# atlas-jj/ORB-SLAM-free-space-carving

Hardware: AMD Instinct MI355X
Metric: Mpix*KF/s fused (640x480xN_KF) (higher is better)
Workload: dtype f32

## Files before the change

orb-slam-free-space-carving_amd/csrc/sdm_device.h:

```cpp
#pragma once
#include <hip/hip_runtime.h>
#include <float.h>
#include <stddef.h>
#include <stdint.h>

#include "sdm_c.h"

namespace sdm {

struct KfMeta {
    float fx, fy, cx, cy;
    float Tcw[12];
    float I_stddev;
    int uploaded;
    int pad[2];
};

struct RefConst {
    int slot;
    float fx, fy, cx, cy;
    float mind, maxd;
    int act_count;
};

// ... 182 lines not shown
    const float u1 = fx * x_min / z_min + cx;
    const float u2 = fx * x_max / z_max + cx;
    const float cols = (float)W;
    const float umin = __builtin_amdgcn_fmed3f(fminf(u1, u2), 0.0f, cols);
    const float umax = __builtin_amdgcn_fmed3f(fmaxf(u1, u2), 0.0f, cols);
    lo = (int)ceilf(umin);
    hi = (int)floorf(umax);
    return !__builtin_isunordered(u1, u2);
}

__device__ __forceinline__ bool gate2_fails_ref(float d, float lambdaL)
{
    if (d >= 360) d -= 360;
    if (d < 0) d += 360;
    if (d > 180) d = 360 - d;
    if (d > 90) d = 180 - d;
    return d > lambdaL;
}
__device__ __forceinline__ bool gate3_fails_ref(float d, float lambdaTheta)
{
    if (d >= 360) d -= 360;
    if (d < 0) d += 360;
    if (d > 180) d = 360 - d;
    return d > lambdaTheta;
}
__device__ __forceinline__ float wrap_neg360(float d)
{
    unsigned neg = (unsigned)((int)__float_as_uint(d) >> 31);
    return d + __uint_as_float(neg & 0x43B40000u);
}
__device__ __forceinline__ bool gate2_fails_fast(float d)
{
    float x = wrap_neg360(d);
    return (fabsf(x - 90.0f) < 10.0f) | (fabsf(x - 270.0f) < 10.0f);
}
__device__ __forceinline__ bool gate3_fails_fast(float d)
{
    float x = wrap_neg360(d);
    return (x > 45.0f) & (x < 315.0f);
}
__device__ __forceinline__ bool gate2_fails_k(float d, float g2c)
{
    const float x = wrap_neg360(d);
    return fabsf(fabsf(x - 180.0f) - 90.0f) < g2c;
}
__device__ __forceinline__ bool gate3_fails_k(float d, unsigned g3lo, unsigned g3span)
{
    const float x = wrap_neg360(d);
    return (__float_as_uint(x) - g3lo) < g3span;
}
__device__ __forceinline__ bool gate2_fails_fast1(float d)
{
    const float x = wrap_neg360(d);
    return fabsf(fabsf(x - 180.0f) - 90.0f) < 10.0f;
}
__device__ __forceinline__ bool gate3_fails_fast1(float d)
{
    const float x = wrap_neg360(d);
    return (__float_as_uint(x) - 0x42340001u) < (0x439D8000u - 0x42340001u);
}

__device__ __forceinline__ float match_cost(float pe2, float ge2, const DevParams& prm)
{
    double s = (double)pe2 + (double)ge2 * prm.inv_theta;
    unsigned lo = (unsigned)__double2loint(s);
    bool risky = (((lo & 0x1FFFFFFFu) - 0x0FFFFF00u) <= 0x200u) | !(s > 1.0e-30) | !(s < 1.0e30);
    if (__builtin_expect(risky, 0)) s = (double)pe2 + (double)ge2 / prm.theta_var;
    return (float)s;
}

#ifndef SDM_ABLATE
#define SDM_ABLATE 0
#endif
#ifndef SDM_SCAN_UNROLL
#define SDM_SCAN_UNROLL 4
#endif
constexpr int SCAN_UNROLL = SDM_SCAN_UNROLL;
typedef float v4f __attribute__((ext_vector_type(4)));

struct SearchStats {
    unsigned long long searches, candidates, gate_pass;
};

__device__ __forceinline__ float rcp_exact(float b)
{
    const float ab = fabsf(b);
    if (__builtin_expect(!((ab >= 0x1p-125f) & (ab < 0x1p125f)), 0)) return 1.0f / b;
    const float r = __builtin_amdgcn_rcpf(b);
    const float e = __builtin_fmaf(-b, r, 1.0f);
    return __builtin_fmaf(e, r, r);
}

#ifndef SDM_K1_OPT_ATAN_RCP
#define SDM_K1_OPT_ATAN_RCP 1
#endif
__device__ __forceinline__ float fast_atan2_deg_x1(float y)
{
    const float scale = (float)(180.0 / 3.14159265358979323846);
    const float p1 = 0.9997878412794807f * scale;
    const float p3 = -0.3258083974640975f * scale;
    const float p5 = 0.1555786518463281f * scale;
    const float p7 = -0.04432655554792128f * scale;
    float ay = fabsf(y);
    float a, c, c2;
    if (1.0f >= ay) {
        c = ay;
        c2 = c * c;
        a = (((p7 * c2 + p5) * c2 + p3) * c2 + p1) * c;
    } else {
#if SDM_K1_OPT_ATAN_RCP
        c = rcp_exact(ay + (float)DBL_EPSILON);
#else
        c = 1.0f / (ay + (float)DBL_EPSILON);
#endif
        c2 = c * c;
        a = 90.f - (((p7 * c2 + p5) * c2 + p3) * c2 + p1) * c;
    }
    if (y < 0) a = 360.f - a;
    return a;
}

#ifndef SDM_K1_OPT
#define SDM_K1_OPT 0x3a27f
#endif

constexpr int PCV_FLOATS = 20;
constexpr int CV_RX = 9, CV_RZ = 12, CV_TX = 15, CV_TZ = 16, CV_ROT = 17, CV_ISTD = 18;
static_assert(offsetof(PairConst, Rx) == 4 * CV_RX && offsetof(PairConst, Rz) == 4 * CV_RZ && offsetof(PairConst, tx) == 4 * CV_TX &&
                  offsetof(PairConst, tz) == 4 * CV_TZ && offsetof(PairConst, rot) == 4 * CV_ROT &&
                  offsetof(PairConst, istd) == 4 * CV_ISTD && offsetof(PairConst, Ry) == 4 * PCV_FLOATS,
              "the CV_* indices follow PairConst");

__device__ __forceinline__ float match_cost1(float pe2, float ge2, const DevParams& prm)
{
    double s = (double)pe2 + (double)ge2 * prm.inv_theta;
    const unsigned lo = (unsigned)__double2loint(s), hi = (unsigned)__double2hiint(s);
    const bool risky = (((lo & 0x1FFFFFFFu) - 0x0FFFFF00u) <= 0x200u) | ((hi - 0x39C00000u) >= (0x46200000u - 0x39C00000u));
    if (__builtin_expect(risky, 0)) s = (double)pe2 + (double)ge2 / prm.theta_var;
    return (float)s;
}

constexpr float INV_THETA_DEFAULT_F = (float)(1.0 / 0.23);
constexpr unsigned COST_BAND = 16u;
__device__ __forceinline__ float match_cost_ref(float pe2, float ge2, const DevParams& prm)
{
    return (float)((double)pe2 + (double)ge2 / prm.theta_var);
}
__device__ __forceinline__ float match_cost_approx(float pe2, float ge2) { return __builtin_fmaf(ge2, INV_THETA_DEFAULT_F, pe2); }

__device__ __forceinline__ float lerp_w0(float yf)
{
#if SDM_K1_OPT & 0x10
    return 1.0f - __builtin_amdgcn_fractf(yf);
#else
    return (floorf(yf) + 1.0f) - yf;
#endif
}
__device__ __forceinline__ float rec_lerp_im_w(const float4& r, float y0w)
{
    unsigned w = __float_as_uint(r.w);
    float y1w = 1.0f - y0w;
    float v0 = (float)(int)(w & 0xffu), v1 = (float)(int)((w >> 8) & 0xffu);
    return v0 * y0w + v1 * y1w;
}
__device__ __forceinline__ float rec_lerp_grad_w(const float4& r, float y0w)
{
    float y1w = 1.0f - y0w;
    return r.x * y0w + r.z * y1w;
}

__device__ __forceinline__ int cvt_i32_sat(float x)
{
    int r;
    asm("v_cvt_i32_f32 %0, %1" : "=v"(r) : "v"(x));
    return r;
}
__device__ __forceinline__ bool search_range_int1(float fx, float cx, float rxxp, float rzxp, float tx, float tz,
                                                  float mind, float maxd, int W, int& lo, int& hi)
{
    float x_min = rxxp * mind + tx, z_min = rzxp * mind + tz;
    float x_max = rxxp * maxd + tx, z_max = rzxp * maxd + tz;
    const float u1 = fx * x_min / z_min + cx;
    const float u2 = fx * x_max / z_max + cx;
    const float mn = __builtin_amdgcn_fmed3f(u1, u2, -__builtin_inff());
    const float mx = __builtin_amdgcn_fmed3f(u1, u2, __builtin_inff());
    lo = min(max(cvt_i32_sat(ceilf(mn)), 0), W);
    hi = min(max(cvt_i32_sat(floorf(mx)), 0), W - 1);
// ... 67 lines not shown
    }
    return ok;
}

struct ScanState {
    float old_err, best_pe, best_ge;
    int best_pixel;
};

struct ScanConst {
    const char* nbase;
    unsigned W16;
    float hlim_b;
    float ab, cb, pixel, grad1, th_line, ang_pi_rot, gate_lim;
    int hi;
};
template <bool STATS, bool CLEAN>
__device__ __forceinline__ void scan_candidate(const ScanConst& q, int uj, float yf, const float4& r, const DevParams& prm,
                                               ScanState& S, SearchStats* st)
{
    if (r.x < prm.lambdaG) return;
#if SDM_ABLATE == 4
    if (r.z > S.old_err) { S.best_pixel = uj; S.old_err = r.z; }
    return;
#endif
    const float d2 = r.y - q.th_line;
    const float d3 = r.y - q.ang_pi_rot;
    bool fail;
    if (CLEAN) {
#if SDM_K1_OPT & 0x04
        fail = gate2_fails_fast1(d2) | gate3_fails_fast1(d3);
#else
        fail = gate2_fails_fast(d2) | gate3_fails_fast(d3);
#endif
    } else {
        fail = gate2_fails_k(d2, prm.g2c) | gate3_fails_k(d3, prm.g3lo, prm.g3span);
        if (__builtin_expect(!((d2 < q.gate_lim) & (d3 < q.gate_lim)), 0))
            fail = gate2_fails_ref(d2, prm.lambdaL) || gate3_fails_ref(d3, prm.lambdaTheta);
    }
    if (fail) return;
    if (STATS) st->gate_pass++;
#if SDM_ABLATE == 3 || SDM_ABLATE == 4
    if (r.z > S.old_err) { S.best_pixel = uj; S.old_err = r.z; }
    return;
#endif
    const float y0w = lerp_w0(yf);
    float pe = q.pixel - rec_lerp_im_w(r, y0w);
    float ge = q.grad1 - rec_lerp_grad_w(r, y0w);
#if SDM_K1_OPT & 0x2000
    if (CLEAN || prm.approx_ok) {
        const float e = CLEAN ? match_cost_approx(pe * pe, ge * ge) : __builtin_fmaf(ge * ge, prm.inv_theta_f, pe * pe);
        bool better = e < S.old_err;
        if (__builtin_expect((__float_as_uint(e) - __float_as_uint(S.old_err) + COST_BAND) <= 2u * COST_BAND, 0))
            better = match_cost_ref(pe * pe, ge * ge, prm) < match_cost_ref(S.best_pe * S.best_pe, S.best_ge * S.best_ge, prm);
        if (better) {
#if SDM_K1_OPT & 0x4000
            asm volatile("" ::: "memory");
#endif
            S.best_pixel = uj;
            S.old_err = e;
            S.best_pe = pe;
            S.best_ge = ge;
        }
        return;
    }
#endif
#if SDM_K1_OPT & 0x08
    float err = match_cost1(pe * pe, ge * ge, prm);
#else
    float err = match_cost(pe * pe, ge * ge, prm);
#endif
    if (err < S.old_err) {
        S.best_pixel = uj;
        S.old_err = err;
        S.best_pe = pe;
        S.best_ge = ge;
    }
}

template <bool STATS, bool CLEAN, int NB>
__device__ __forceinline__ void scan_batch(const ScanConst& q, int u0, float u0f, const DevParams& prm, ScanState& S,
                                           SearchStats* st)
{
    float yfs[NB];
    unsigned long long rowok[NB];
    v4f rs[NB];
    const unsigned c0 = (unsigned)u0 << 4;
#if !(SDM_K1_OPT & 0x01)
    const unsigned hi16 = (unsigned)max(q.hi, 0) << 4;
#endif
#pragma unroll
    for (int k = 0; k < NB; k++) {
        float yf = -(q.ab * (u0f + (float)k) + q.cb);
        float yc = __builtin_amdgcn_fmed3f(yf, 1.0f, q.hlim_b);
#if SDM_K1_OPT & 0x01
        const unsigned off = __umul24((unsigned)(int)yc, q.W16) + c0;
        const char* __restrict__ nb_k = q.nbase + 16 * k;
#else
        unsigned uc16 = min(c0 + 16u * k, hi16);
        unsigned off = __umul24((unsigned)(int)yc, q.W16) + uc16;
        const char* __restrict__ nb_k = q.nbase;
#endif
        yfs[k] = yf;
        rowok[k] = __builtin_amdgcn_fcmpf(yc, yf, 1 );
#if SDM_ABLATE == 5
        rs[k] = v4f{20.0f + (float)(off & 15u), 10.0f, 21.0f, __uint_as_float(0x6040u)};
#else
        rs[k] = *reinterpret_cast<const v4f*>(nb_k + off);
#endif
    }
#pragma unroll
    for (int k = 0; k < NB; k++)
        asm volatile("" : "+v"(rs[k]));
#pragma unroll
    for (int k = 0; k < NB; k++) {
        const int uj = u0 + k;
        if (STATS && uj <= q.hi) st->candidates++;
        const float4 r = make_float4(rs[k].x, rs[k].y, rs[k].z, rs[k].w);
        if (!((uj <= q.hi) & __builtin_amdgcn_inverse_ballot_w64(rowok[k]))) continue;
        scan_candidate<STATS, CLEAN>(q, uj, yfs[k], r, prm, S, st);
    }
}

template <bool STATS, bool CLEAN>
__device__ __forceinline__ void scan_segment(const ScanConst& q, int lo, const DevParams& prm, ScanState& S, SearchStats* st)
{
    float u0f = (float)lo;
    for (int u0 = lo; u0 <= q.hi; u0 += SCAN_UNROLL, u0f += (float)SCAN_UNROLL)
        scan_batch<STATS, CLEAN, SCAN_UNROLL>(q, u0, u0f, prm, S, st);
}

#ifndef SDM_MASK_MIN_L
#define SDM_MASK_MIN_L 24
#endif
#ifndef SDM_MASK_MIN_L_UNION
#define SDM_MASK_MIN_L_UNION 48
#endif
#ifndef SDM_MASK_MAX_SLOPE
#define SDM_MASK_MAX_SLOPE 0.25f
#endif
#ifndef SDM_MASK_NB
#define SDM_MASK_NB 2
#endif
#ifndef SDM_MASK_BINS
#define SDM_MASK_BINS 1
#endif
constexpr int MASK_BINS = 16;
constexpr int MASK_WINDOW = 6;
constexpr int MASK_UNION = MASK_BINS + MASK_WINDOW - 1;
constexpr int MASK_PLANES = MASK_UNION + 1;
constexpr unsigned MASK_WORD_BYTES = 4u * MASK_PLANES;
constexpr float MASK_EPS = 0x1p-6f;
constexpr int MASK_HINT_L = SDM_MASK_MIN_L * 3 / 4;
#ifndef SDM_MASK_CALL_MEAN_L
#define SDM_MASK_CALL_MEAN_L 32
#endif
constexpr int MASK_CALL_MEAN_L = SDM_MASK_CALL_MEAN_L;
constexpr float MASK_ANG_MARGIN = 0.01f;
constexpr float MASK_MAX_LAMBDA_THETA = 56.0f;
constexpr float MASK_BIN_SCALE = (float)MASK_BINS / 360.0f;
__host__ __device__ __forceinline__ int mask_bin(float t)
{
    const int b = (int)(t * MASK_BIN_SCALE);
    return b < MASK_BINS - 1 ? b : MASK_BINS - 1;
}
struct MaskStats {
    unsigned long long waves, steps, row_mismatch;
};
struct MaskView {
    const char* base;
    unsigned row_pitch;
};
template <bool STATS, bool CLEAN, bool BINNED>
__device__ __forceinline__ void scan_masked(const ScanConst& q, const MaskView& mv, int lo, const DevParams& prm, ScanState& S,
                                            SearchStats* st, MaskStats* ms)
{
    const float yh = -(q.ab * (float)q.hi + q.cb);
    const float inv_s = __builtin_amdgcn_rcpf(fabsf(q.ab)) * 0.998046875f;
    const bool falling = q.ab > 0.0f;
    unsigned pl0 = 4u * (unsigned)MASK_UNION;
    if (BINNED) {
        float w0 = q.ang_pi_rot - (prm.lambdaTheta + MASK_ANG_MARGIN);
        if (w0 < 0.0f) w0 += 360.0f;
        pl0 = 4u * (unsigned)mask_bin(w0);
    }
    for (int base = lo; base <= q.hi; base += 64) {
        const int chi = min(q.hi, base + 63);
        unsigned long long cand = 0ull;
        bool ended = false;
        int u = base;
        while (u <= chi) {
            const float yf = -(q.ab * (float)u + q.cb);
            const float yc = __builtin_amdgcn_fmed3f(yf, 1.0f, q.hlim_b);
            if (!(yc == yf)) {
                const bool out_lo = (yf < 1.0f) & (yh < 1.0f), out_hi = (yf > q.hlim_b) & (yh > q.hlim_b);
                if (!(yf == yf) | out_lo | out_hi) {
                    if (STATS) st->candidates += (unsigned long long)(q.hi - u + 1);
                    ended = true;
                    break;
                }
                if (STATS) st->candidates++;
                u++;
                continue;
            }
            const float fr = __builtin_amdgcn_fractf(yf);
            const float room = (falling ? fr : 1.0f - fr) - MASK_EPS;
            const int n = max(cvt_i32_sat(room * inv_s), 0);
            const int cover = min(min(n, chi - u), 32);
            const char* __restrict__ mp = mv.base + (__umul24((unsigned)(int)yc, mv.row_pitch) + __umul24((unsigned)u >> 5, MASK_WORD_BYTES) + pl0);
            unsigned mlo, mhi;
            if (BINNED) {
                typedef unsigned mword4 __attribute__((ext_vector_type(4), aligned(4)));
                typedef unsigned mword2 __attribute__((ext_vector_type(2), aligned(4)));
                const mword4 a0 = *reinterpret_cast<const mword4*>(mp);
                const mword2 a1 = *reinterpret_cast<const mword2*>(mp + 16);
                const mword4 b0 = *reinterpret_cast<const mword4*>(mp + MASK_WORD_BYTES);
                const mword2 b1 = *reinterpret_cast<const mword2*>(mp + MASK_WORD_BYTES + 16);
                mlo = (a0.x | a0.y | a0.z) | (a0.w | a1.x | a1.y);
                mhi = (b0.x | b0.y | b0.z) | (b0.w | b1.x | b1.y);
            } else {
                mlo = *reinterpret_cast<const unsigned*>(mp);
                mhi = *reinterpret_cast<const unsigned*>(mp + MASK_WORD_BYTES);
            }
            unsigned long long bits = (((unsigned long long)mhi << 32) | (unsigned long long)mlo) >> ((unsigned)u & 31u);
            bits &= (2ull << cover) - 1ull;
            cand |= bits << (unsigned)(u - base);
            if (STATS) {
                st->candidates += (unsigned long long)(cover + 1);
                ms->steps++;
            }
            u += cover + 1;
        }
        if (STATS) {
            for (int k = 0; base + k <= (ended ? u - 1 : chi); k++) {
                const float yk = -(q.ab * (float)(base + k) + q.cb);
                if (!(__builtin_amdgcn_fmed3f(yk, 1.0f, q.hlim_b) == yk)) continue;
                const v4f r = *reinterpret_cast<const v4f*>(q.nbase + (__umul24((unsigned)(int)yk, q.W16) + ((unsigned)(base + k) << 4)));
                if (r.x < prm.lambdaG) continue;
                const bool fail = gate2_fails_ref(r.y - q.th_line, prm.lambdaL) || gate3_fails_ref(r.y - q.ang_pi_rot, prm.lambdaTheta);
                if (!fail && !((cand >> k) & 1ull)) ms->row_mismatch++;
            }
        }
        while (cand != 0ull) {
            int ujs[SDM_MASK_NB];
            float yfs[SDM_MASK_NB];
            v4f rs[SDM_MASK_NB];
            unsigned long long okm[SDM_MASK_NB];
#pragma unroll
            for (int k = 0; k < SDM_MASK_NB; k++) {
                okm[k] = __builtin_amdgcn_ballot_w64(cand != 0ull);
                const int uj = base + (cand != 0ull ? (int)__builtin_ctzll(cand) : 0);
                cand &= cand - 1ull;
                const float yfj = -(q.ab * (float)uj + q.cb);
                const float ycj = __builtin_amdgcn_fmed3f(yfj, 1.0f, q.hlim_b);
                ujs[k] = uj;
                yfs[k] = yfj;
                rs[k] = *reinterpret_cast<const v4f*>(q.nbase + (__umul24((unsigned)(int)ycj, q.W16) + ((unsigned)uj << 4)));
            }
#pragma unroll
            for (int k = 0; k < SDM_MASK_NB; k++)
                asm volatile("" : "+v"(rs[k]));
#pragma unroll
            for (int k = 0; k < SDM_MASK_NB; k++) {
                if (!__builtin_amdgcn_inverse_ballot_w64(okm[k])) continue;
                scan_candidate<STATS, CLEAN>(q, ujs[k], yfs[k], make_float4(rs[k].x, rs[k].y, rs[k].z, rs[k].w), prm, S, st);
            }
        }
        if (ended) break;
    }
}

__device__ __forceinline__ int wave_max_nonneg(int v)
{
    v = max(v, __builtin_amdgcn_update_dpp(0, v, 0x111, 0xf, 0xf, false));
    v = max(v, __builtin_amdgcn_update_dpp(0, v, 0x112, 0xf, 0xf, false));
    v = max(v, __builtin_amdgcn_update_dpp(0, v, 0x114, 0xf, 0xf, false));
    v = max(v, __builtin_amdgcn_update_dpp(0, v, 0x118, 0xf, 0xf, false));
    v = max(v, __builtin_amdgcn_update_dpp(0, v, 0x142, 0xa, 0xf, false));
    v = max(v, __builtin_amdgcn_update_dpp(0, v, 0x143, 0xc, 0xf, false));
    return __builtin_amdgcn_readlane(v, 63);
}
template <bool STATS, bool CLEAN>
__device__ __forceinline__ void scan_planned(const ScanConst& q, int lo, int Lmax, const DevParams& prm, ScanState& S,
                                             SearchStats* st)
{
    int n3 = (-Lmax) & 3;
    if (Lmax <= 3) n3 = 1;
    if (Lmax == 5) n3 = 2;
    const int n4 = max(Lmax - 3 * n3, 0) >> 2;
    int u0 = lo;
    float u0f = (float)lo;
    for (int i = 0; i < n4; i++, u0 += 4, u0f += 4.0f)
        if (u0 <= q.hi) scan_batch<STATS, CLEAN, 4>(q, u0, u0f, prm, S, st);
    for (int i = 0; i < n3; i++, u0 += 3, u0f += 3.0f)
        if (u0 <= q.hi) scan_batch<STATS, CLEAN, 3>(q, u0, u0f, prm, S, st);
}

template <bool STATS, bool PLAN = false, bool MASK = false>
__device__ __forceinline__ bool epipolar_search(const float4* __restrict__ nrec, int W, int H,
                                                const float* __restrict__ cv, const float* __restrict__ rcv, int clean,
                                                bool on, int x, int y, float pixel, float grad1,
                                                float th_pi, float xp0, float xp1, const DevParams& prm, float& rho_o,
                                                float& sigma_o, float& best_u, float& best_v,
                                                SearchStats* st, const MaskView mv = MaskView{nullptr, 0u}, MaskStats* ms = nullptr)
{
    float fx = rcv[0], cx = rcv[1];
    const float mind = rcv[2], maxd = rcv[3];
    rho_o = 0.f;
    sigma_o = 0.f;
    best_u = 0.f;
    best_v = 0.f;
    if (STATS && on) st->searches++;
    const float* F = cv;
    float a = (float)x * F[0] + (float)y * F[3] + F[6];
    float b = (float)x * F[1] + (float)y * F[4] + F[7];
    float c = (float)x * F[2] + (float)y * F[5] + F[8];
#if SDM_K1_OPT & 0x8000
    float ab, cb;
    if (clean & 2) {
        const float rb = rcp_fast(b);
        ab = quot_fast(a, b, rb);
        cb = quot_fast(c, b, rb);
    } else {
        ab = a / b;
        cb = c / b;
    }
    bool live = on & (ab >= -4) & (ab <= 4);
    if (!PLAN && !live) return false;
#else
    float ab = a / b;
    bool live = on & (ab >= -4) & (ab <= 4);
    if (!PLAN && !live) return false;
    float cb = c / b;
#endif

    float rxxp = row_dot_xp(cv + CV_RX, xp0, xp1);
    float rzxp = row_dot_xp(cv + CV_RZ, xp0, xp1);
    float tx = cv[CV_TX], tz = cv[CV_TZ];
    int lo, hi;
#if SDM_K1_OPT & 0x20
    live &= search_range_int1(fx, cx, rxxp, rzxp, tx, tz, mind, maxd, W, lo, hi);
#else
    live &= search_range_int(fx, cx, rxxp, rzxp, tx, tz, mind, maxd, W, lo, hi);
    if (hi > W - 1) hi = W - 1;
#endif
    if (!PLAN && !live) return false;

    float th_line = fast_atan2_deg_x1(-ab);
    float ang_pi_rot = wrap_once_360(th_pi + cv[CV_ROT]);

    const float gate_lim = prm.closed_ok ? 360.0f : -__builtin_inff();
    ScanState S = {1000000.0f, 1000.0f, 0.f, -1};
    const float hlim2 = (float)(H - 2);
    const char* __restrict__ nbase = reinterpret_cast<const char*>(nrec);
#if SDM_ABLATE == 10
    if (ang_pi_rot + th_line + (float)(hi - lo) != 12345.678f) live = false;
#endif
#if SDM_ABLATE == 11
    if (ab + cb + rxxp + rzxp != 12345.678f) live = false;
#endif
#if SDM_ABLATE == 6
    hi = lo - 1;
    S.old_err = ab;
    S.best_pixel = lo + 2;
#endif
    if (PLAN && !live) hi = lo - 1;
    ScanConst sc;
    sc.nbase = nbase;
    sc.W16 = (unsigned)W << 4;
    sc.hlim_b = __uint_as_float(__float_as_uint((float)(H - 1)) - 1u);
    sc.ab = ab;
    sc.cb = cb;
    sc.pixel = pixel;
    sc.grad1 = grad1;
    sc.th_line = th_line;
    sc.ang_pi_rot = ang_pi_rot;
    sc.gate_lim = gate_lim;
    sc.hi = hi;
    if (PLAN) {
        const int Lmax = wave_max_nonneg(max(hi - lo + 1, 0));
        if (Lmax > 0) {
#if SDM_K1_OPT & 0x02
            if ((clean & 1) && prm.default_gates && prm.fast_theta_div)
                scan_planned<STATS, true>(sc, lo, Lmax, prm, S, st);
            else
#endif
                scan_planned<STATS, false>(sc, lo, Lmax, prm, S, st);
        }
        if (!live) return false;
    } else {
        bool masked = false;
        const unsigned long long here = __builtin_amdgcn_ballot_w64(true);
#ifndef SDM_MASK_DISABLE
        if (MASK && mv.base != nullptr && prm.scan_mode != 1 && ((clean & 4) || prm.scan_mode == 2)) {
            const bool binned = (clean & 1) && prm.bins_ok && SDM_MASK_BINS;
            const int min_l = binned ? SDM_MASK_MIN_L : SDM_MASK_MIN_L_UNION;
            const unsigned long long lng = __builtin_amdgcn_ballot_w64(hi - lo + 1 >= min_l);
            const unsigned long long steep = __builtin_amdgcn_ballot_w64(fabsf(ab) > SDM_MASK_MAX_SLOPE);
            masked = prm.scan_mode == 2 || (2 * __popcll(lng) >= __popcll(here) && steep == 0ull);
        }
#endif
        if (MASK && masked) {
            if (STATS && (int)__builtin_amdgcn_mbcnt_hi(~0u, __builtin_amdgcn_mbcnt_lo(~0u, 0u)) == (int)__builtin_ctzll(here)) ms->waves++;
#if SDM_K1_OPT & 0x02
            if ((clean & 1) && prm.default_gates && prm.fast_theta_div)
                scan_masked<STATS, true, SDM_MASK_BINS != 0>(sc, mv, lo, prm, S, st, ms);
            else
#endif
                if ((clean & 1) && prm.bins_ok && SDM_MASK_BINS)
                scan_masked<STATS, false, true>(sc, mv, lo, prm, S, st, ms);
            else
                scan_masked<STATS, false, false>(sc, mv, lo, prm, S, st, ms);
        } else {
#if SDM_K1_OPT & 0x02
            if ((clean & 1) && prm.default_gates && prm.fast_theta_div)
                scan_segment<STATS, true>(sc, lo, prm, S, st);
            else
#endif
                scan_segment<STATS, false>(sc, lo, prm, S, st);
        }
    }
    const float best_pe = S.best_pe, best_ge = S.best_ge;
    const int best_pixel = S.best_pixel;
    if (best_pixel < 0) return false;
#if SDM_ABLATE == 2
    rho_o = S.old_err + best_pe + (float)best_pixel;
    sigma_o = best_ge + 1.0f;
    return true;
#endif


    int up = best_pixel + 1, um = best_pixel - 1;
    if (um < 0 || up > W - 1) return false;
    float yfp = -(ab * (float)up + cb);
    float yfm = -(ab * (float)um + cb);
    float fyp = floorf(yfp), fym = floorf(yfm);
    if (!(fyp >= 0.0f && fyp <= hlim2)) return false;
    if (!(fym >= 0.0f && fym <= hlim2)) return false;
    int y0p = (int)fyp, y0m = (int)fym;
#if SDM_K1_OPT & 0x20000
    v4f vp = *reinterpret_cast<const v4f*>(nbase + ((__umul24((unsigned)y0p, (unsigned)W) + (unsigned)up) << 4));
    v4f vm = *reinterpret_cast<const v4f*>(nbase + ((__umul24((unsigned)y0m, (unsigned)W) + (unsigned)um) << 4));
    asm volatile("" : "+v"(vp));
    asm volatile("" : "+v"(vm));
    const float4 rp = make_float4(vp.x, vp.y, vp.z, vp.w), rm = make_float4(vm.x, vm.y, vm.z, vm.w);
#else
    float4 rp = *reinterpret_cast<const float4*>(nbase + ((__umul24((unsigned)y0p, (unsigned)W) + (unsigned)up) << 4));
    float4 rm = *reinterpret_cast<const float4*>(nbase + ((__umul24((unsigned)y0m, (unsigned)W) + (unsigned)um) << 4));
#endif
    const float y1p = fyp + 1.0f, y1m = fym + 1.0f;
    float g = (rec_lerp_im(rp, y1p, yfp) - rec_lerp_im(rm, y1m, yfm)) / 2;
    float q = (rec_lerp_grad(rp, y1p, yfp) - rec_lerp_grad(rm, y1m, yfm)) / 2;
    const double inv_theta = prm.inv_theta;
    float gg = g * g;
    float denom = (float)((double)gg + inv_theta * (double)q * (double)q);
    float gpe = g * best_pe;
    float ustar = (float)((double)best_pixel +
                          ((double)gpe + inv_theta * (double)q * (double)best_ge) / (double)denom);
    float ustar_var = 2 * cv[CV_ISTD] * cv[CV_ISTD] / denom;
    best_u = ustar;
    best_v = -(ab * ustar + cb);

    float d0 = pixel_depth(ustar, fx, cx, rzxp, rxxp, tx, tz);
    float s = sqrt_exact(ustar_var);
    float dmin = pixel_depth(ustar - s, fx, cx, rzxp, rxxp, tx, tz);
    float dmax = pixel_depth(ustar + s, fx, cx, rzxp, rxxp, tx, tz);
    float e1 = fabsf(dmax - d0), e2 = fabsf(dmin - d0);
    rho_o = d0;
    sigma_o = (e1 < e2) ? e2 : e1;
    return true;
}

__device__ __forceinline__ bool chi_test(float a, float b, float sa, float sb)
{
    float d = a - b;
    float num = d * d;
    float chi = num / (sa * sa) + num / (sb * sb);
    return (double)chi < 5.99;
}

__device__ __forceinline__ double div_by_with_rcp(double a, double b, double r)
{
    double q0 = a * r;
    double e0 = __builtin_fma(-q0, b, a);
    double q1 = __builtin_fma(e0, r, q0);
    double e1 = __builtin_fma(-q1, b, a);
    return __builtin_fma(e1, r, q1);
}
__device__ __forceinline__ void fusion_terms(float rho, float sg, double& t_rho, double& t_one)
{
    double s2 = (double)sg * (double)sg;
    const float ar = fabsf(rho);
#if SDM_K1_OPT & 512
    const unsigned hi = (unsigned)__double2hiint(s2);
    const bool safe = ((hi - 0x39B00000u) < (0x46400000u - 0x39B00000u)) & (ar > 1.0e-30f) & (ar < 1.0e30f);
    if (safe) {
        double y = (double)__builtin_amdgcn_rcpf(sg * sg);
        double e = __builtin_fma(-s2, y, 1.0);
        y = __builtin_fma(e, y, y);
        e = __builtin_fma(-s2, y, 1.0);
        y = __builtin_fma(e, y, y);
        e = __builtin_fma(-s2, y, 1.0);
        t_one = __builtin_fma(e, y, y);
        t_rho = div_by_with_rcp((double)rho, s2, t_one);
    } else {
        t_one = 1.0 / s2;
        t_rho = (double)rho / s2;
    }
#else
    t_one = 1.0 / s2;
    const bool safe = (s2 > 1.0e-60) & (s2 < 1.0e60) & (ar > 1.0e-30f) & (ar < 1.0e30f);
    t_rho = safe ? div_by_with_rcp((double)rho, s2, t_one) : (double)rho / s2;
#endif
}
__device__ __forceinline__ void fusion_accum(float rho, float sg, float& pjsj, float& rsj)
{
    double t_rho, t_one;
    fusion_terms(rho, sg, t_rho, t_one);
    pjsj = (float)((double)pjsj + t_rho);
    rsj = (float)((double)rsj + t_one);
}

__device__ __forceinline__ bool gt_1em6(float x) { return x > __uint_as_float(0x358637bdu); }
__device__ __forceinline__ bool lt_1em6(float x) { return x <= __uint_as_float(0x358637bdu); }

__device__ __forceinline__ float safe_rcp_sq(float s)
{
    float s2 = s * s;
    bool ok = (s2 >= 1.0e-30f) && (s2 <= 1.0e30f);
    return ok ? __builtin_amdgcn_rcpf(s2) : __builtin_nanf("");
}

__device__ __forceinline__ bool chi_test_fast(float a, float b, float sa, float sb, float ra, float rb)
{
    float d = a - b;
    float num = d * d;
    float approx = num * ra + num * rb;
    if (approx < 5.9896f) return true;
    if (approx > 5.9904f) return false;
    return chi_test(a, b, sa, sb);
}

__device__ __forceinline__ bool chi_test_lazy(float2 ha, float2 hb, float sa, const float* sb_ptr)
{
// ... 41 lines not shown
```

orb-slam-free-space-carving_amd/csrc/sdm_kernels.h:

```cpp
#pragma once
#include "sdm_device.h"
#include "sdm_ingest.h"

namespace sdm {

#ifndef SDM_INTRA_COMPACT
#define SDM_INTRA_COMPACT 1
#endif

struct TileGeom {
    int W, H, tiles_x, tiles_y, ntiles;
};

__host__ __device__ inline TileGeom make_geom(int W, int H)
{
    TileGeom g;
    g.W = W;
    g.H = H;
    g.tiles_x = (W + TILE_W - 1) / TILE_W;
    g.tiles_y = (H + TILE_H - 1) / TILE_H;
    g.ntiles = g.tiles_x * g.tiles_y;
    return g;
}
__host__ inline int grid_blocks(const TileGeom& g, int n_ref) { return 8 * ((g.ntiles + 7) / 8) * n_ref; }
// ... 218 lines not shown
        const int a = K1_WAVES * i + ((i & 1) ? (K1_WAVES - 1 - w) : w);
        if (a >= n || !((vm >> a) & 1ull)) continue;
        const float2 ha = hyp[a * K1_PX + p];
        const float sa = sgm[a * K1_PX + p];
        unsigned c = (sa * sa > 0.0f) ? 1u : 0u;
        for (int bb = a + 1; bb < n; bb++) {
            const float2 hb = hyp[bb * K1_PX + p];
            if (chi_test_lazy(ha, hb, sa, &sgm[bb * K1_PX + p])) {
                c++;
                atomicAdd(&cnt[(bb >> 2) * K1_PX + p], 1u << (8 * (bb & 3)));
            }
        }
        atomicAdd(&cnt[(a >> 2) * K1_PX + p], c << (8 * (a & 3)));
    }
}
__device__ __forceinline__ bool k1_fuse_counted(const float2* hyp, const float* sgm, const unsigned* cnt, unsigned long long vm,
                                                int n, int p, int lambdaN, float2& result)
{
    unsigned best = 0;
    int besta = 0;
    for (int a = 0; a < n; a++) {
        if (!((vm >> a) & 1ull)) continue;
        const unsigned c = (cnt[(a >> 2) * K1_PX + p] >> (8 * (a & 3))) & 0xffu;
        if (c > best) {
            best = c;
            besta = a;
        }
    }
    if ((int)best < lambdaN) return false;
    const float2 ha = hyp[besta * K1_PX + p];
    const float sa = sgm[besta * K1_PX + p];
    float pjsj = 0.f, rsj = 0.f;
    for (int bb = 0; bb < n; bb++) {
        if (!((vm >> bb) & 1ull)) continue;
        const float2 hb = hyp[bb * K1_PX + p];
        const bool in = (bb == besta) ? (sa * sa > 0.0f) : chi_test_lazy(ha, hb, sa, &sgm[bb * K1_PX + p]);
        if (in) fusion_accum(hb.x, sgm[bb * K1_PX + p], pjsj, rsj);
    }
    result = make_float2(pjsj / rsj, sqrtf(1 / rsj));
    return true;
}

#ifndef SDM_K1_EU_MIN
#define SDM_K1_EU_MIN 8
#endif
#ifndef SDM_K1_LB
#define SDM_K1_LB __launch_bounds__(K1_BLOCK) __attribute__((amdgpu_waves_per_eu(SDM_K1_EU_MIN, 8)))
#endif
template <bool STATS, bool MASK>
__global__ SDM_K1_LB void k_search_fuse(const float4* __restrict__ rec, long long plane,
                                                       const RefConst* __restrict__ refs,
                                                       const PairConst* __restrict__ pairs, int n_ref, int n,
                                                       int W, int H, int max_chunks, DevParams prm,
                                                       const unsigned* __restrict__ act, float2* __restrict__ pool,
                                                       unsigned long long* __restrict__ stats, OpenList open_list,
                                                       const unsigned* __restrict__ gmask, int mrow)
{
    extern __shared__ __align__(16) unsigned char smem_raw[];
    float2* hyp = reinterpret_cast<float2*>(smem_raw);
    float* sgm = reinterpret_cast<float*>(hyp + (size_t)n * K1_PX);
    unsigned* cnt = reinterpret_cast<unsigned*>(sgm + (size_t)n * K1_PX);
    const int cnt_words = max((n + 3) >> 2, K1_OUTLIER_ROWS);
    unsigned long long* pmask = reinterpret_cast<unsigned long long*>(cnt + (size_t)cnt_words * K1_PX);
    unsigned long long* set0 = pmask + K1_BLOCK;
    unsigned* cnt0 = reinterpret_cast<unsigned*>(set0 + K1_PX);
    unsigned* xbase = cnt0 + K1_PX;

    const int b = blockIdx.x;
    const int i8 = b >> 3;
    const int cl = i8 / n_ref;
    const int ref = i8 - cl * n_ref;
    const int chunk = cl * 8 + (b & 7);
    if (chunk >= max_chunks) return;
    const RefConst rc = refs[ref];
    if (chunk * K1_PX >= rc.act_count) return;
    const int tid = threadIdx.x, p = tid & (K1_PX - 1);
    const int w = __builtin_amdgcn_readfirstlane(tid >> 6);
    const int t = chunk * K1_PX + p;
    const bool on = t < rc.act_count;
    const float4* __restrict__ rrec = rec + (long long)rc.slot * plane;

    int x = 2, y = 2;
    float pixel = 0.f, grad1 = 0.f, th_pi = 0.f, xp0 = 0.f, xp1 = 0.f;
    if (on) {
        unsigned xy = act[(long long)rc.slot * plane + t];
        x = (int)(xy & 0xffffu);
        y = (int)(xy >> 16);
        float4 r = rrec[y * W + x];
        pixel = (float)(int)(__float_as_uint(r.w) & 0xffu);
        grad1 = r.x;
        th_pi = r.y;
        xp0 = ((float)x - rc.cx) / rc.fx;
        xp1 = ((float)y - rc.cy) / rc.fy;
    }
    SearchStats st = {0, 0, 0};
    MaskStats ms = {0, 0, 0};
    MaskView mv;
    mv.row_pitch = (unsigned)mrow * MASK_WORD_BYTES;
    const PairConst* __restrict__ pcs = pairs + (long long)ref * n;
    const float rcvb[4] = {rc.fx, rc.cx, rc.mind, rc.maxd};
    const float* __restrict__ rcv = rcvb;
    unsigned long long mymask = 0;
    for (int j = w; j < n; j += K1_WAVES) {
        const PairConst* __restrict__ pc = pcs + j;
        const float4* __restrict__ nrec = rec + (long long)pc->nbr_slot * plane;
        float2 h = make_float2(__builtin_inff(), 1.0f);
#if SDM_K1_OPT & 0x1000
        {
            float rho, sigma, bu, bv;
            const float* __restrict__ cv = reinterpret_cast<const float*>(pc);
            bool ok = epipolar_search<STATS, true>(nrec, W, H, cv, rcv, pc->clean, on, x, y, pixel, grad1, th_pi, xp0, xp1, prm,
                                                   rho, sigma, bu, bv, &st);
            if (ok && __float_as_uint(rho) < 0x7f800000u) {
                h = make_float2(rho, sigma);
                mymask |= 1ull << j;
            }
        }
#else
        if (on) {
            float rho, sigma, bu, bv;
            const float* __restrict__ cv = reinterpret_cast<const float*>(pc);
            mv.base = (MASK && gmask) ? reinterpret_cast<const char*>(gmask + (long long)pc->nbr_slot * H * MASK_PLANES * mrow) : nullptr;
            bool ok = epipolar_search<STATS, false, MASK>(nrec, W, H, cv, rcv, pc->clean, true, x, y, pixel, grad1, th_pi, xp0, xp1, prm, rho,
                                             sigma, bu, bv, &st, mv, &ms);
            if (ok && __float_as_uint(rho) < 0x7f800000u) {
                h = make_float2(rho, sigma);
                mymask |= 1ull << j;
            }
        }
#endif
        hyp[j * K1_PX + p] = make_float2(h.x, safe_rcp_sq(h.y));
        sgm[j * K1_PX + p] = h.y;
    }
    for (int q = w; q < cnt_words; q += K1_WAVES) cnt[q * K1_PX + p] = 0u;
    if (w == 0) {
        set0[p] = 0ull;
        cnt0[p] = 0u;
    }
    pmask[tid] = mymask;
    __syncthreads();

    unsigned long long vm = 0;
#pragma unroll
    for (int q = 0; q < K1_WAVES; q++) vm |= pmask[q * K1_PX + p];
#if SDM_ABLATE == 1
    const int nh = 0;
    if (vm == 0x123456789ull) pool[0] = make_float2(1.f, 1.f);
#else
    const int nh = __popcll(vm);
#endif
    const bool go = nh > prm.lambdaN;
    const int a0 = (int)__ffsll((long long)vm) - 1;
    bool self0 = false;
    if (go) {
        const float2 ha = hyp[a0 * K1_PX + p];
        const float sa = sgm[a0 * K1_PX + p];
        self0 = sa * sa > 0.0f;
        unsigned c = 0;
        for (int bb = w; bb < n; bb += K1_WAVES) {
            const float2 hb = hyp[bb * K1_PX + p];
            if (bb != a0 && chi_test_lazy(ha, hb, sa, &sgm[bb * K1_PX + p])) c++;
        }
        if (c) atomicAdd(&cnt0[p], c);
    }
    __syncthreads();
#if SDM_ABLATE == 9
    bool settled = false;
    const bool few = false;
    const unsigned long long S0 = 0ull;
    const int s0 = 0;
#else
    bool settled = go && self0 && (int)cnt0[p] + 1 == nh;
    const bool more = go && !settled && self0;
    unsigned long long S0 = settled ? vm : 0ull;
    if (__builtin_amdgcn_ballot_w64(more) != 0ull) {
        if (more) {
            const float2 ha = hyp[a0 * K1_PX + p];
            const float sa = sgm[a0 * K1_PX + p];
            unsigned long long m = 0;
            for (int bb = w; bb < n; bb += K1_WAVES) {
                const float2 hb = hyp[bb * K1_PX + p];
                if (bb != a0 && chi_test_lazy(ha, hb, sa, &sgm[bb * K1_PX + p])) m |= 1ull << bb;
            }
            if (m) atomicOr(&set0[p], m);
        }
        __syncthreads();
        if (more) S0 = set0[p] | (1ull << a0);
    }
    const int s0 = __popcll(S0);
    const unsigned long long O = vm & ~S0;
    const bool few = more && __popcll(O) <= K1_OUTLIER_ROWS;
    if (__builtin_amdgcn_ballot_w64(few) != 0ull) {
        unsigned* orow = cnt;
        unsigned long long rem = few ? O : 0ull;
        for (int i = 0; i < K1_OUTLIER_ROWS && __builtin_amdgcn_ballot_w64(rem != 0ull) != 0ull; i++) {
            if (rem != 0ull) {
                const int o = (int)__ffsll((long long)rem) - 1;
                rem &= rem - 1ull;
                const float2 ho = hyp[o * K1_PX + p];
                const float so = sgm[o * K1_PX + p];
                unsigned c = (w == 0 && so * so > 0.0f) ? 1u : 0u;
                for (int bb = w; bb < n; bb += K1_WAVES) {
                    const float2 hb = hyp[bb * K1_PX + p];
                    if (bb != o && chi_test_lazy(ho, hb, so, &sgm[bb * K1_PX + p])) c += ((S0 >> bb) & 1ull) ? 0x10001u : 1u;
                }
                if (c) atomicAdd(&orow[i * K1_PX + p], c);
            }
        }
        __syncthreads();
        if (few) {
            bool stands = true;
            const int nO = __popcll(O);
            for (int i = 0; i < K1_OUTLIER_ROWS; i++) {
                const unsigned v = orow[i * K1_PX + p];
                if (i < nO) stands = stands && (v >> 16) == 0u && (int)(v & 0xffffu) <= s0;
            }
            settled = stands;
        }
        __syncthreads();
        for (int q = w; q < K1_OUTLIER_ROWS; q += K1_WAVES) cnt[q * K1_PX + p] = 0u;
    }
#endif
    const bool open = go && !settled;
    const unsigned long long open_mask = __builtin_amdgcn_ballot_w64(open);
    bool deferred = false;
    if (open_mask != 0ull) {
        if (tid == 0) {
            const unsigned cntw = (unsigned)__popcll(open_mask);
            unsigned first = 0xFFFFFFFFu;
            if (cntw < open_list.inplace_min && atomicAdd(&open_list.count[0], cntw) >= open_list.quota) {
                const unsigned base = atomicAdd(&open_list.count[2], cntw);
                if (base <= open_list.capacity && cntw <= open_list.capacity - base)
                    first = base;
                else
                    atomicMin(&open_list.count[1], base);
            }
            xbase[0] = first;
        }
        __syncthreads();
        const unsigned base = xbase[0];
        deferred = base != 0xFFFFFFFFu;
        if (deferred) {
            if (open) {
                const unsigned e = base + (unsigned)__popcll(open_mask & ((1ull << p) - 1ull));
                float2* __restrict__ dst = open_list.hyp + ((size_t)(e >> 6) * n) * K1_PX + (e & 63u);
                for (int j = w; j < n; j += K1_WAVES) dst[(size_t)j * K1_PX] = make_float2(hyp[j * K1_PX + p].x, sgm[j * K1_PX + p]);
                if (w == 0) {
                    open_list.pix[e] = (long long)rc.slot * plane + y * W + x;
                    open_list.vm[e] = vm;
                }
            }
        } else {
            if (open) k1_count_all_pairs(hyp, sgm, cnt, vm, n, p, w);
            __syncthreads();
        }
    }

    unsigned long long n_fused = 0;
    if (w == 0 && on && !(open && deferred)) {
        float2 result = make_float2(0.f, 0.f);
        if (settled) {
            if (s0 >= prm.lambdaN) {
                float pjsj = 0.f, rsj = 0.f;
                for (int bb = 0; bb < n; bb++) {
                    if (!((S0 >> bb) & 1ull)) continue;
                    fusion_accum(hyp[bb * K1_PX + p].x, sgm[bb * K1_PX + p], pjsj, rsj);
                }
                result = make_float2(pjsj / rsj, sqrtf(1 / rsj));
                n_fused = 1;
            }
        } else if (go) {
            n_fused = k1_fuse_counted(hyp, sgm, cnt, vm, n, p, prm.lambdaN, result) ? 1 : 0;
        }
        pool[(long long)rc.slot * plane + y * W + x] = result;
    }
    if (STATS) {
        unsigned long long v[9] = {st.searches, st.candidates, st.gate_pass,
                                   (w == 0 && on) ? (unsigned long long)nh : 0ull, n_fused, ms.waves, ms.steps, ms.row_mismatch,
                                   (w == 0 && open) ? 1ull : 0ull};
#pragma unroll
        for (int k = 0; k < 9; k++) {
            unsigned long long s = v[k];
            for (int o = 32; o > 0; o >>= 1) s += __shfl_down(s, o);
            if ((tid & 63) == 0 && s) atomicAdd(&stats[k], s);
        }
    }
}

template <bool STATS>
__global__ __launch_bounds__(K1_BLOCK) void k_fuse_open(OpenList open_list, int n, DevParams prm, float2* __restrict__ pool,
                                                        long long pool_elems, unsigned long long* __restrict__ stats)
{
    extern __shared__ __align__(16) unsigned char smem_raw[];
    float2* hyp = reinterpret_cast<float2*>(smem_raw);
    float* sgm = reinterpret_cast<float*>(hyp + (size_t)n * K1_PX);
    unsigned* cnt = reinterpret_cast<unsigned*>(sgm + (size_t)n * K1_PX);
    const int cnt_words = (n + 3) >> 2;
    const unsigned total = min(min(open_list.count[2], open_list.count[1]), open_list.capacity);
    const int tid = threadIdx.x, p = tid & (K1_PX - 1);
    if (blockIdx.x == 0 && tid == 0) {
        open_list.next[0] = 0u;
        open_list.next[1] = 0xFFFFFFFFu;
        open_list.next[2] = 0u;
    }
    const int w = __builtin_amdgcn_readfirstlane(tid >> 6);
    unsigned long long n_fused = 0;
    for (unsigned blk = blockIdx.x; blk * (unsigned)K1_PX < total; blk += gridDim.x) {
        const unsigned e = blk * K1_PX + p;
        const bool on = e < total;
        const float2* __restrict__ src = open_list.hyp + ((size_t)blk * n) * K1_PX + p;
        for (int j = w; j < n; j += K1_WAVES) {
            const float2 h = on ? src[(size_t)j * K1_PX] : make_float2(__builtin_inff(), 1.0f);
            hyp[j * K1_PX + p] = make_float2(h.x, safe_rcp_sq(h.y));
            sgm[j * K1_PX + p] = h.y;
        }
        for (int q = w; q < cnt_words; q += K1_WAVES) cnt[q * K1_PX + p] = 0u;
        const unsigned long long vm = on ? open_list.vm[e] : 0ull;
        __syncthreads();
        if (on) k1_count_all_pairs(hyp, sgm, cnt, vm, n, p, w);
        __syncthreads();
        if (w == 0 && on) {
            float2 result = make_float2(0.f, 0.f);
            if (k1_fuse_counted(hyp, sgm, cnt, vm, n, p, prm.lambdaN, result)) n_fused++;
            const long long px = open_list.pix[e];
            if (px >= 0 && px < pool_elems) pool[px] = result;
        }
        __syncthreads();
    }
    if (STATS) {
        for (int o = 32; o > 0; o >>= 1) n_fused += __shfl_down(n_fused, o);
        if ((tid & 63) == 0 && n_fused) atomicAdd(&stats[4], n_fused);
    }
}

constexpr int HALO_W = TILE_W + 2;
constexpr int HALO_H = TILE_H + 2;
__device__ __forceinline__ void load_halo(const float2* __restrict__ in, int W, int H, int tx0, int ty0,
                                          float2* tile)
{
    for (int i = threadIdx.x; i < HALO_W * HALO_H; i += BLOCK) {
        int hy = i / HALO_W, hx = i - hy * HALO_W;
        int x = tx0 + hx - 1, y = ty0 + hy - 1;
        float2 v = make_float2(0.f, 0.f);
        if (x >= 0 && x < W && y >= 0 && y < H) v = in[y * W + x];
        tile[i] = v;
    }
}

__global__ __launch_bounds__(BLOCK) void k_intra_check(const float2* __restrict__ in_base, float2* __restrict__ out_base,
                                                       const long long* __restrict__ in_off,
                                                       const long long* __restrict__ out_off, int n_ref, TileGeom g)
{
    __shared__ float2 tile[HALO_W * HALO_H];
    __shared__ float2 outv[TILE_PX];
    __shared__ unsigned short act[TILE_PX];
    __shared__ int wsum[16];
    int ref, tx0, ty0;
    if (!decode_block(g, n_ref, ref, tx0, ty0)) return;
// ... 1311 lines not shown
```

Before: 13810.

## Flatten epipolar search setup and refine to reduce wave divergence

Makes the per-pair epipolar search setup branch-free. Lanes no longer return early when inactive. They carry a live flag, get an empty range, and the whole wave exits only when a ballot shows no live lanes. The atan2 helper computes the shallow-slope polynomial for every lane and runs the reciprocal branch only when some lane needs it. The sub-pixel refine bounds checks and the result store become predicated selects. The aim is to cut divergent control flow and exec-mask churn on the GPU, at the cost of extra arithmetic on lanes that are inactive or out of range. Optional asm phase markers are added for profiling.

Measured after the change: 13870 (median of 6 runs). No clear change (+0.4%).

```diff
diff --git a/orb-slam-free-space-carving_amd/csrc/sdm_device.h b/orb-slam-free-space-carving_amd/csrc/sdm_device.h
--- a/orb-slam-free-space-carving_amd/csrc/sdm_device.h
+++ b/orb-slam-free-space-carving_amd/csrc/sdm_device.h
@@ -288,6 +288,18 @@
     unsigned long long searches, candidates, gate_pass;
 };
 
+#ifndef SDM_K1_FLAT_SETUP
+#define SDM_K1_FLAT_SETUP 1
+#endif
+#ifndef SDM_K1_FLAT_REFINE
+#define SDM_K1_FLAT_REFINE 1
+#endif
+#ifdef SDM_K1_MARKERS
+#define SDM_K1_PHASE(name) asm volatile("; K1_PHASE " name)
+#else
+#define SDM_K1_PHASE(name) ((void)0)
+#endif
+
 __device__ __forceinline__ float rcp_exact(float b)
 {
     const float ab = fabsf(b);
@@ -309,6 +321,25 @@
     const float p7 = -0.04432655554792128f * scale;
     float ay = fabsf(y);
     float a, c, c2;
+#if SDM_K1_FLAT_SETUP
+    c = ay;
+    c2 = c * c;
+    a = (((p7 * c2 + p5) * c2 + p3) * c2 + p1) * c;
+    const bool steep = !(1.0f >= ay);
+    if (__builtin_amdgcn_ballot_w64(steep) != 0ull) {
+        if (steep) {
+#if SDM_K1_OPT_ATAN_RCP
+            c = rcp_exact(ay + (float)DBL_EPSILON);
+#else
+            c = 1.0f / (ay + (float)DBL_EPSILON);
+#endif
+            c2 = c * c;
+            a = 90.f - (((p7 * c2 + p5) * c2 + p3) * c2 + p1) * c;
+        }
+    }
+    if (y < 0) a = 360.f - a;
+    return a;
+#endif
     if (1.0f >= ay) {
         c = ay;
         c2 = c * c;
@@ -542,6 +573,7 @@
 __device__ __forceinline__ void scan_batch(const ScanConst& q, int u0, float u0f, const DevParams& prm, ScanState& S,
                                            SearchStats* st)
 {
+    if constexpr (CLEAN) SDM_K1_PHASE("scan-batch-clean"); else SDM_K1_PHASE("scan-batch-other");
     float yfs[NB];
     unsigned long long rowok[NB];
     v4f rs[NB];
@@ -635,6 +667,7 @@
 __device__ __forceinline__ void scan_masked(const ScanConst& q, const MaskView& mv, int lo, const DevParams& prm, ScanState& S,
                                             SearchStats* st, MaskStats* ms)
 {
+    SDM_K1_PHASE("scan-masked");
     const float yh = -(q.ab * (float)q.hi + q.cb);
     const float inv_s = __builtin_amdgcn_rcpf(fabsf(q.ab)) * 0.998046875f;
     const bool falling = q.ab > 0.0f;
@@ -771,6 +804,8 @@
     best_u = 0.f;
     best_v = 0.f;
     if (STATS && on) st->searches++;
+    constexpr bool FLAT = PLAN || SDM_K1_FLAT_SETUP;
+    SDM_K1_PHASE("line");
     const float* F = cv;
     float a = (float)x * F[0] + (float)y * F[3] + F[6];
     float b = (float)x * F[1] + (float)y * F[4] + F[7];
@@ -786,14 +821,15 @@
         cb = c / b;
     }
     bool live = on & (ab >= -4) & (ab <= 4);
-    if (!PLAN && !live) return false;
+    if (!FLAT && !live) return false;
 #else
     float ab = a / b;
     bool live = on & (ab >= -4) & (ab <= 4);
-    if (!PLAN && !live) return false;
+    if (!FLAT && !live) return false;
     float cb = c / b;
 #endif
 
+    SDM_K1_PHASE("range");
     float rxxp = row_dot_xp(cv + CV_RX, xp0, xp1);
     float rzxp = row_dot_xp(cv + CV_RZ, xp0, xp1);
     float tx = cv[CV_TX], tz = cv[CV_TZ];
@@ -804,8 +840,10 @@
     live &= search_range_int(fx, cx, rxxp, rzxp, tx, tz, mind, maxd, W, lo, hi);
     if (hi > W - 1) hi = W - 1;
 #endif
-    if (!PLAN && !live) return false;
-
+    if (!FLAT && !live) return false;
+    if (FLAT && !PLAN && __builtin_amdgcn_ballot_w64(live) == 0ull) return false;
+
+    SDM_K1_PHASE("angle");
     float th_line = fast_atan2_deg_x1(-ab);
     float ang_pi_rot = wrap_once_360(th_pi + cv[CV_ROT]);
 
@@ -824,7 +862,7 @@
     S.old_err = ab;
     S.best_pixel = lo + 2;
 #endif
-    if (PLAN && !live) hi = lo - 1;
+    if (FLAT && !live) hi = lo - 1;
     ScanConst sc;
     sc.nbase = nbase;
     sc.W16 = (unsigned)W << 4;
@@ -837,6 +875,7 @@
     sc.ang_pi_rot = ang_pi_rot;
     sc.gate_lim = gate_lim;
     sc.hi = hi;
+    SDM_K1_PHASE("scan");
     if (PLAN) {
         const int Lmax = wave_max_nonneg(max(hi - lo + 1, 0));
         if (Lmax > 0) {
@@ -850,13 +889,13 @@
         if (!live) return false;
     } else {
         bool masked = false;
-        const unsigned long long here = __builtin_amdgcn_ballot_w64(true);
+        const unsigned long long here = __builtin_amdgcn_ballot_w64(live);
 #ifndef SDM_MASK_DISABLE
         if (MASK && mv.base != nullptr && prm.scan_mode != 1 && ((clean & 4) || prm.scan_mode == 2)) {
             const bool binned = (clean & 1) && prm.bins_ok && SDM_MASK_BINS;
             const int min_l = binned ? SDM_MASK_MIN_L : SDM_MASK_MIN_L_UNION;
             const unsigned long long lng = __builtin_amdgcn_ballot_w64(hi - lo + 1 >= min_l);
-            const unsigned long long steep = __builtin_amdgcn_ballot_w64(fabsf(ab) > SDM_MASK_MAX_SLOPE);
+            const unsigned long long steep = __builtin_amdgcn_ballot_w64(live & (fabsf(ab) > SDM_MASK_MAX_SLOPE));
             masked = prm.scan_mode == 2 || (2 * __popcll(lng) >= __popcll(here) && steep == 0ull);
         }
 #endif
@@ -880,8 +919,17 @@
                 scan_segment<STATS, false>(sc, lo, prm, S, st);
         }
     }
+    SDM_K1_PHASE("refine");
     const float best_pe = S.best_pe, best_ge = S.best_ge;
     const int best_pixel = S.best_pixel;
+#if SDM_K1_FLAT_REFINE && SDM_ABLATE != 2
+    const int up = best_pixel + 1, um = best_pixel - 1;
+    const float yfp = -(ab * (float)up + cb);
+    const float yfm = -(ab * (float)um + cb);
+    const float fyp = floorf(yfp), fym = floorf(yfm);
+    const bool refine = (um >= 0) & (up <= W - 1) & (fyp >= 0.0f) & (fyp <= hlim2) & (fym >= 0.0f) & (fym <= hlim2);
+    if (!refine) return false;
+#else
     if (best_pixel < 0) return false;
 #if SDM_ABLATE == 2
     rho_o = S.old_err + best_pe + (float)best_pixel;
@@ -897,6 +945,7 @@
     float fyp = floorf(yfp), fym = floorf(yfm);
     if (!(fyp >= 0.0f && fyp <= hlim2)) return false;
     if (!(fym >= 0.0f && fym <= hlim2)) return false;
+#endif
     int y0p = (int)fyp, y0m = (int)fym;
 #if SDM_K1_OPT & 0x20000
     v4f vp = *reinterpret_cast<const v4f*>(nbase + ((__umul24((unsigned)y0p, (unsigned)W) + (unsigned)up) << 4));
@@ -920,6 +969,7 @@
     float ustar_var = 2 * cv[CV_ISTD] * cv[CV_ISTD] / denom;
     best_u = ustar;
     best_v = -(ab * ustar + cb);
+    SDM_K1_PHASE("depth");
 
     float d0 = pixel_depth(ustar, fx, cx, rzxp, rxxp, tx, tz);
     float s = sqrt_exact(ustar_var);
diff --git a/orb-slam-free-space-carving_amd/csrc/sdm_kernels.h b/orb-slam-free-space-carving_amd/csrc/sdm_kernels.h
--- a/orb-slam-free-space-carving_amd/csrc/sdm_kernels.h
+++ b/orb-slam-free-space-carving_amd/csrc/sdm_kernels.h
@@ -324,6 +324,9 @@
 
     int x = 2, y = 2;
     float pixel = 0.f, grad1 = 0.f, th_pi = 0.f, xp0 = 0.f, xp1 = 0.f;
+#if SDM_K1_FLAT_SETUP && !(SDM_K1_OPT & 0x1000)
+    xp0 = __builtin_nanf("");
+#endif
     if (on) {
         unsigned xy = act[(long long)rc.slot * plane + t];
         x = (int)(xy & 0xffffu);
@@ -344,6 +347,7 @@
     const float* __restrict__ rcv = rcvb;
     unsigned long long mymask = 0;
     for (int j = w; j < n; j += K1_WAVES) {
+        SDM_K1_PHASE("pair");
         const PairConst* __restrict__ pc = pcs + j;
         const float4* __restrict__ nrec = rec + (long long)pc->nbr_slot * plane;
         float2 h = make_float2(__builtin_inff(), 1.0f);
@@ -358,6 +362,25 @@
                 mymask |= 1ull << j;
             }
         }
+#elif SDM_K1_FLAT_SETUP
+        {
+            float rho, sigma, bu, bv;
+            const float* __restrict__ cv = reinterpret_cast<const float*>(pc);
+            mv.base = (MASK && gmask) ? reinterpret_cast<const char*>(gmask + (long long)pc->nbr_slot * H * MASK_PLANES * mrow) : nullptr;
+            const bool ok = epipolar_search<STATS, false, MASK>(nrec, W, H, cv, rcv, pc->clean, STATS ? on : true, x, y, pixel, grad1, th_pi, xp0, xp1, prm,
+                                                                rho, sigma, bu, bv, &st, mv, &ms);
+            SDM_K1_PHASE("store");
+#if SDM_K1_FLAT_REFINE
+            const bool take = ok & (__float_as_uint(rho) < 0x7f800000u);
+            h = make_float2(take ? rho : __builtin_inff(), take ? sigma : 1.0f);
+            mymask |= take ? (1ull << j) : 0ull;
+#else
+            if (ok && __float_as_uint(rho) < 0x7f800000u) {
+                h = make_float2(rho, sigma);
+                mymask |= 1ull << j;
+            }
+#endif
+        }
 #else
         if (on) {
             float rho, sigma, bu, bv;
@@ -365,15 +388,23 @@
             mv.base = (MASK && gmask) ? reinterpret_cast<const char*>(gmask + (long long)pc->nbr_slot * H * MASK_PLANES * mrow) : nullptr;
             bool ok = epipolar_search<STATS, false, MASK>(nrec, W, H, cv, rcv, pc->clean, true, x, y, pixel, grad1, th_pi, xp0, xp1, prm, rho,
                                              sigma, bu, bv, &st, mv, &ms);
+            SDM_K1_PHASE("store");
+#if SDM_K1_FLAT_REFINE
+            const bool take = ok & (__float_as_uint(rho) < 0x7f800000u);
+            h = make_float2(take ? rho : __builtin_inff(), take ? sigma : 1.0f);
+            mymask |= take ? (1ull << j) : 0ull;
+#else
             if (ok && __float_as_uint(rho) < 0x7f800000u) {
                 h = make_float2(rho, sigma);
                 mymask |= 1ull << j;
             }
+#endif
         }
 #endif
         hyp[j * K1_PX + p] = make_float2(h.x, safe_rcp_sq(h.y));
         sgm[j * K1_PX + p] = h.y;
     }
+    SDM_K1_PHASE("fusion-bounds");
     for (int q = w; q < cnt_words; q += K1_WAVES) cnt[q * K1_PX + p] = 0u;
     if (w == 0) {
         set0[p] = 0ull;
@@ -498,6 +529,7 @@
         }
     }
 
+    SDM_K1_PHASE("getfusion");
     unsigned long long n_fused = 0;
     if (w == 0 && on && !(open && deferred)) {
         float2 result = make_float2(0.f, 0.f);
@@ -506,8 +538,10 @@
                 float pjsj = 0.f, rsj = 0.f;
                 for (int bb = 0; bb < n; bb++) {
                     if (!((S0 >> bb) & 1ull)) continue;
+                    SDM_K1_PHASE("getfusion-term");
                     fusion_accum(hyp[bb * K1_PX + p].x, sgm[bb * K1_PX + p], pjsj, rsj);
                 }
+                SDM_K1_PHASE("getfusion-result");
                 result = make_float2(pjsj / rsj, sqrtf(1 / rsj));
                 n_fused = 1;
             }
@@ -516,6 +550,7 @@
         }
         pool[(long long)rc.slot * plane + y * W + x] = result;
     }
+    SDM_K1_PHASE("end");
     if (STATS) {
         unsigned long long v[9] = {st.searches, st.candidates, st.gate_pass,
                                    (w == 0 && on) ? (unsigned long long)nh : 0ull, n_fused, ms.waves, ms.steps, ms.row_mismatch,
```
